# librosa/librosa

Measured on NVIDIA H100. Metric: mel-spectrogram frames/sec (n_fft=2048,hop=512,n_mels=128), higher is better.
Workload: dtype f32

## Files before the change

include/b2l.h:

```cpp
#ifndef B2L_H_
#define B2L_H_

#include <stddef.h>
#include <stdint.h>

#ifdef __cplusplus
extern "C" {
#endif

#define B2L_VERSION 100

enum b2l_status {
  B2L_OK = 0,
  B2L_ERR_INVALID = 1,
  B2L_ERR_CUDA = 2,
  B2L_ERR_UNSUPPORTED = 3,
  B2L_ERR_OOM = 4,
  B2L_ERR_NCCL = 5
};

enum b2l_pad_mode {
  B2L_PAD_CONSTANT = 0,
  B2L_PAD_EDGE = 1,
  B2L_PAD_REFLECT = 2,
// ... 30 lines not shown
int b2l_ctx_destroy(b2l_ctx* ctx);
int b2l_ctx_sync(b2l_ctx* ctx);
int b2l_ctx_device(const b2l_ctx* ctx, int* device);
int b2l_ctx_sm_count(const b2l_ctx* ctx, int* sms);
int b2l_ctx_launch_count(const b2l_ctx* ctx, uint64_t* launches);

int b2l_status_reset(b2l_ctx* ctx);
int b2l_status_read(b2l_ctx* ctx, int* status);
int b2l_scan_finite(b2l_ctx* ctx, const float* d_y, int64_t n_clips, int64_t n, int64_t y_stride,
                    int64_t begin);
int b2l_scan_finite_f64(b2l_ctx* ctx, const double* d_y, int64_t n_clips, int64_t n, int64_t y_stride,
                        int64_t begin);

int b2l_alloc(b2l_ctx* ctx, size_t bytes, void** d_ptr);
int b2l_free(b2l_ctx* ctx, void* d_ptr);
int b2l_memset(b2l_ctx* ctx, void* d_ptr, int value, size_t bytes);
int b2l_h2d(b2l_ctx* ctx, void* d_dst, const void* h_src, size_t bytes);
int b2l_d2h(b2l_ctx* ctx, void* h_dst, const void* d_src, size_t bytes);
int b2l_d2d(b2l_ctx* ctx, void* d_dst, const void* d_src, size_t bytes);
int b2l_copy2d(b2l_ctx* ctx, void* d_dst, size_t dst_pitch, const void* d_src, size_t src_pitch, size_t width_bytes,
               size_t rows);
int b2l_host_alloc(size_t bytes, void** h_ptr);
int b2l_host_free(void* h_ptr);
int b2l_mem_info(b2l_ctx* ctx, size_t* free_bytes, size_t* total_bytes);

int b2l_event_create(b2l_ctx* ctx, b2l_event** ev);
int b2l_event_record(b2l_ctx* ctx, b2l_event* ev);
int b2l_event_elapsed_ms(b2l_event* start, b2l_event* stop, float* ms);
int b2l_event_destroy(b2l_event* ev);

int b2l_plan_create(b2l_ctx* ctx, const b2l_plan_desc* desc, b2l_plan** plan);
int b2l_plan_destroy(b2l_plan* plan);
int b2l_plan_n_frames(const b2l_plan* plan, int64_t n, int64_t* n_frames);


int b2l_stft(b2l_ctx* ctx, const b2l_plan* plan, const float* d_y, int64_t n_clips, int64_t n,
             int64_t y_stride, void* d_D );

int b2l_spectrogram(b2l_ctx* ctx, const b2l_plan* plan, const float* d_y, int64_t n_clips, int64_t n,
                    int64_t y_stride, float* d_S);

int b2l_melspectrogram(b2l_ctx* ctx, const b2l_plan* plan, const float* d_y, int64_t n_clips, int64_t n,
                       int64_t y_stride, float* d_mel);

int b2l_mfcc(b2l_ctx* ctx, const b2l_plan* plan, const float* d_y, int64_t n_clips, int64_t n,
             int64_t y_stride, float* d_mfcc, float* d_logmel);

int b2l_istft(b2l_ctx* ctx, const b2l_plan* plan, const void* d_D, int64_t n_clips, int64_t n_frames_stored,
              int64_t n_frames_used, const float* d_inv_wss, int64_t out_len, float* d_y, int64_t y_stride);

int b2l_mel_project(b2l_ctx* ctx, const b2l_plan* plan, const float* d_S, int64_t n_clips,
                    int64_t n_frames, float* d_mel);
int b2l_power_to_db(b2l_ctx* ctx, const float* d_in, int64_t n_clips, int64_t per_clip, float amin,
                    float ref_value, float top_db, float* d_out);
typedef struct b2l_onset_desc {
  int32_t lag, max_size, pad_width, detrend, n_channels;
  int32_t bounds[33];
} b2l_onset_desc;
int b2l_onset_from_spec(b2l_ctx* ctx, const b2l_onset_desc* desc, const float* d_S, int64_t n_clips, int64_t n_rows,
                        int64_t n_frames, float* d_out);
int b2l_onset_median_from_spec(b2l_ctx* ctx, const b2l_onset_desc* desc, const float* d_S, int64_t n_clips,
                               int64_t n_rows, int64_t n_frames, float* d_out);
typedef struct b2l_pcen_desc {
  float gain, bias, power, eps, b;
  int32_t max_size;
} b2l_pcen_desc;
// ... 193 lines not shown
```

librosa_b200/_native.py:

```python
from __future__ import annotations

import ctypes as C
import os
import threading
import weakref
from typing import Optional, Tuple

import numpy as np

_HERE = os.path.dirname(os.path.abspath(__file__))
LIB_PATH = os.environ.get("B2L_LIB_PATH") or os.path.join(_HERE, "csrc", "libb2l.so")

B2L_OK = 0
B2L_ERR_INVALID = 1
B2L_ERR_CUDA = 2
B2L_ERR_UNSUPPORTED = 3
B2L_ERR_OOM = 4
B2L_ERR_NCCL = 5

PAD_MODES = {"constant": 0, "edge": 1, "reflect": 2, "symmetric": 3, "linear_ramp": 4, "empty": 5}


class NativeLibraryError(RuntimeError):
    """libb2l.so is missing / failed, or a CUDA / NCCL call failed."""
# ... 130 lines not shown
def _declare(lib):
    P = C.POINTER
    sig = {
        "b2l_version": (C.c_int, []),
        "b2l_last_error": (C.c_char_p, []),
        "b2l_device_count": (C.c_int, [P(C.c_int)]),
        "b2l_ctx_create": (C.c_int, [C.c_int, P(_vp)]),
        "b2l_ctx_destroy": (C.c_int, [_vp]),
        "b2l_ctx_sync": (C.c_int, [_vp]),
        "b2l_ctx_device": (C.c_int, [_vp, P(C.c_int)]),
        "b2l_ctx_sm_count": (C.c_int, [_vp, P(C.c_int)]),
        "b2l_ctx_launch_count": (C.c_int, [_vp, P(C.c_uint64)]),
        "b2l_status_reset": (C.c_int, [_vp]),
        "b2l_status_read": (C.c_int, [_vp, P(C.c_int)]),
        "b2l_scan_finite": (C.c_int, [_vp, _vp, _i64, _i64, _i64, _i64]),
        "b2l_scan_finite_f64": (C.c_int, [_vp, _vp, _i64, _i64, _i64, _i64]),
        "b2l_alloc": (C.c_int, [_vp, C.c_size_t, P(_vp)]),
        "b2l_free": (C.c_int, [_vp, _vp]),
        "b2l_memset": (C.c_int, [_vp, _vp, C.c_int, C.c_size_t]),
        "b2l_h2d": (C.c_int, [_vp, _vp, _vp, C.c_size_t]),
        "b2l_d2h": (C.c_int, [_vp, _vp, _vp, C.c_size_t]),
        "b2l_d2d": (C.c_int, [_vp, _vp, _vp, C.c_size_t]),
        "b2l_copy2d": (C.c_int, [_vp, _vp, C.c_size_t, _vp, C.c_size_t, C.c_size_t, C.c_size_t]),
        "b2l_host_alloc": (C.c_int, [C.c_size_t, P(_vp)]),
        "b2l_host_free": (C.c_int, [_vp]),
        "b2l_mem_info": (C.c_int, [_vp, P(C.c_size_t), P(C.c_size_t)]),
        "b2l_event_create": (C.c_int, [_vp, P(_vp)]),
        "b2l_event_record": (C.c_int, [_vp, _vp]),
        "b2l_event_elapsed_ms": (C.c_int, [_vp, _vp, P(C.c_float)]),
        "b2l_event_destroy": (C.c_int, [_vp]),
        "b2l_plan_create": (C.c_int, [_vp, P(PlanDesc), P(_vp)]),
        "b2l_plan_destroy": (C.c_int, [_vp]),
        "b2l_plan_n_frames": (C.c_int, [_vp, _i64, P(_i64)]),
        "b2l_stft": (C.c_int, [_vp, _vp, _vp, _i64, _i64, _i64, _vp]),
        "b2l_spectrogram": (C.c_int, [_vp, _vp, _vp, _i64, _i64, _i64, _vp]),
        "b2l_melspectrogram": (C.c_int, [_vp, _vp, _vp, _i64, _i64, _i64, _vp]),
        "b2l_mfcc": (C.c_int, [_vp, _vp, _vp, _i64, _i64, _i64, _vp, _vp]),
        "b2l_istft": (C.c_int, [_vp, _vp, _vp, _i64, _i64, _i64, _vp, _i64, _vp, _i64]),
        "b2l_mel_project": (C.c_int, [_vp, _vp, _vp, _i64, _i64, _vp]),
        "b2l_power_to_db": (C.c_int, [_vp, _vp, _i64, _i64, C.c_float, C.c_float, C.c_float, _vp]),
        "b2l_onset_from_spec": (C.c_int, [_vp, P(OnsetDesc), _vp, _i64, _i64, _i64, _vp]),
        "b2l_onset_median_from_spec": (C.c_int, [_vp, P(OnsetDesc), _vp, _i64, _i64, _i64, _vp]),
        "b2l_pcen": (C.c_int, [_vp, P(PcenDesc), _vp, _i64, _i64, _i64, _vp, _vp, _vp, _vp]),
        "b2l_resample_poly": (C.c_int, [_vp, _vp, _i64, _i64, _i64, _vp, C.c_int32, C.c_int32, C.c_int32, _i64, _i64, _i64,
                                        C.c_float, _vp]),
        "b2l_spectral_contrast": (C.c_int, [_vp, P(ContrastDesc), _vp, _i64, _i64, C.c_int32, _vp, _vp]),
        "b2l_sub": (C.c_int, [_vp, _vp, _vp, _i64, _vp]),
        "b2l_pip_pass": (C.c_int, [_vp, P(PipDesc), _vp, _i64, C.c_int32, _vp, _vp]),
        "b2l_normalize_rows": (C.c_int, [_vp, _vp, _i64, _i64, _i64, C.c_int32, C.c_float, _vp]),
        "b2l_hpss": (C.c_int, [_vp, P(HpssDesc), _vp, _vp, _i64, _i64, _i64, _vp, _vp]),
        "b2l_cabs": (C.c_int, [_vp, _vp, _i64, _vp]),
        "b2l_reassign": (C.c_int, [_vp, P(ReassignDesc), _vp, _vp, _vp, _i64, _i64, _i64, _vp, _vp, _vp, _vp, _vp]),
        "b2l_phase_vocoder": (C.c_int, [_vp, _vp, _i64, _i64, _i64, _i64, _vp, _vp, _vp, _vp, _vp]),
        "b2l_unary": (C.c_int, [_vp, C.c_int32, _vp, _i64, C.c_float, _vp]),
        "b2l_dct_project": (C.c_int, [_vp, _vp, _vp, _i64, _i64, _vp]),
        "b2l_transpose": (C.c_int, [_vp, _vp, _i64, _i64, _i64, C.c_int32, _vp]),
        "b2l_gl_update": (C.c_int, [_vp, _vp, _vp, _vp, C.c_float, C.c_float, _vp, _i64]),
        "b2l_spectral_stats": (C.c_int, [_vp, _vp, P(StatsDesc), _vp, _i64, _i64, _i64, _vp, _vp]),
        "b2l_spectral_stats_from_spec": (C.c_int, [_vp, P(StatsDesc), _vp, _i64, _i64, C.c_int32, _vp, _vp]),
        "b2l_frame_feature": (C.c_int, [_vp, C.c_int32, _vp, _i64, _i64, _i64, C.c_int32, C.c_int32, C.c_int32,
                                        C.c_int32, C.c_float, C.c_int32, C.c_int32, C.c_float, _vp]),
        "b2l_yin_cmnd": (C.c_int, [_vp, P(YinDesc), _vp, _i64, _i64, _i64, _vp]),
        "b2l_yin_pick": (C.c_int, [_vp, P(YinDesc), _vp, _i64, _vp]),
        "b2l_pyin_obs": (C.c_int, [_vp, P(PyinDesc), _vp, _i64, _vp, _vp, _vp, _vp]),
        "b2l_viterbi": (C.c_int, [_vp, P(PyinDesc), _vp, _vp, _vp, _vp, _i64, _i64, _vp, _vp, _vp]),
        "b2l_tempogram": (C.c_int, [_vp, P(TempogramDesc), _vp, _i64, _i64, _vp, _vp]),
# ... 447 lines not shown
```

librosa_b200/csrc/api.cu:

```cuda
#include <cuda_runtime.h>
#include <math.h>
#include <stdlib.h>
#include <string.h>

#include <algorithm>

#include "aux_kernels.cuh"
#include "czt_kernel.cuh"
#include "feat_kernels.cuh"
#include "internal.h"
#include "mr_kernel.cuh"
#include "pitch_kernels.cuh"

using namespace b2l;

#define B2L_CASE(L) case L: return fwd_kernel_##L(variant, mode);
static FwdKernel fwd_kernel_for(int log2m, int variant, int mode) {
  switch (log2m) { B2L_FFT_SIZES(B2L_CASE) }
  return nullptr;
}
#undef B2L_CASE
#define B2L_CASE(L) case L: return inv_kernel_##L(variant);
static InvKernel inv_kernel_for(int log2m, int variant) {
  switch (log2m) { B2L_FFT_SIZES(B2L_CASE) }
  return nullptr;
}
#undef B2L_CASE
#define B2L_CASE(L) case L: return czt_kernel_##L();
static CztKernel czt_kernel_for(int log2p) {
  switch (log2p) { B2L_CZT_SIZES(B2L_CASE) }
  return nullptr;
}
#undef B2L_CASE
#define B2L_CASE(L) case L: return czt_inv_kernel_##L();
static CztInvKernel czt_inv_kernel_for(int log2p) {
  switch (log2p) { B2L_CZT_SIZES(B2L_CASE) }
  return nullptr;
}
#undef B2L_CASE

static int cta_variants(const HostFftCfg& cfg, int out[3]) {
  int n = 0;
  if (cfg.log2m >= 9 && cfg.log2m <= 11) out[n++] = 116;
  int nws[2];
  const int k = cfg.nw_options(nws);
  for (int i = 0; i < k; ++i) out[n++] = nws[i];
  return n;
}
static int variant_threads(int variant) { return variant == 116 ? 512 : variant * 32; }

// ... 79 lines not shown
    off += (size_t)a.in_stride * nh;
    a.off_xbuf = (int)(off = align_up(off, 128));
    size_t xbytes = (size_t)f * cfg.xbuf_f2() * 8;
    if (mode == MODE_MEL || mode == MODE_STATS) {
      xbytes = (size_t)f * mel_group_stride(M, f) * 8 + (M < 128 ? (size_t)(M + 16) * 4 : 0);
    }
    a.xbuf_stride = (int)align_up(xbytes, 128);
    off += (size_t)a.xbuf_stride * nh;
    if (off > c->smem_optin) continue;
    variant = v;
    ft = f;
    halves = nh;
    smem = off;
    rt = t;
    a.in_floats = (int)span;
  }
  if (!variant)
    return fail(B2L_ERR_UNSUPPORTED, "hop_length=%d with n_fft=%d needs more shared memory than one SM has", p->hop,
                p->n_fft);

  a.y = d_y;
  a.clip_stride = y_stride;
  a.n = (int)n;
  a.n_clips = (int)n_clips;
  a.n_fft = N;
  a.hop = p->hop;
  a.pad = p->center ? N / 2 : 0;
  a.pad_mode = p->pad_mode;
  a.n_frames = (int)T;
  a.tiles_per_clip = (int)((T + ft - 1) / ft);
  a.total_tiles = (long long)a.tiles_per_clip * n_clips;
  a.tma_ok = (((uintptr_t)d_y & 15) == 0) && (y_stride % 4 == 0) && (a.in_floats % 4 == 0);
  a.window = p->d_win_fwd;
  a.tw = p->d_tw_fwd;
  a.twn = p->d_twn;
  a.out_c = out_c;
  a.out_r = out_r;
  a.power_mode = p->power_mode;
  a.power = p->power;
  a.n_mels = p->n_mels;
  if (mode == MODE_STATS) {
    if (!stats || !stats->d_freq) return fail(B2L_ERR_INVALID, "NULL frequency table");
    a.power_mode = 1;
    a.power = 1.0f;
    a.stats = stats->sp;
    a.mel_w = stats->d_freq;
    a.mel_w_count = M + 1;
  }
  if (rt) {
    a.mel_w_count = rt->w_count;
    a.mel_w = rt->d_w;
    a.mel_rows = rt->d_rows;
    a.n_mel_rows = rt->n_rows;
  }
  a.log_mode = log_mode ? 1 : 0;
  a.out_tiled = log_mode == 2 ? 1 : 0;
  a.amin = p->amin;
  a.db_sub = 10.0f * log10f(fmaxf(p->amin, fabsf(p->ref_value)));
  a.clip_max = c->d_clip_max;
  a.status = c->d_status;

  const FwdKernel fn = fwd_kernel_for(p->log2m, variant, mode);
  if (!fn) return fail(B2L_ERR_CUDA, "no forward kernel variant %d for n_fft=%d", variant, N);
  const int threads = variant_threads(variant);
  long long grid = 0;
  if ((rc = resident_grid(c, fn, threads, smem, (a.total_tiles + halves - 1) / halves, &grid))) return rc;
  if (!grid) return fail(B2L_ERR_CUDA, "forward kernel does not fit on an SM (smem %zu)", smem);
  return launch(c, fn, (unsigned)grid, threads, smem, a);
}

static size_t czt_smem(const b2l_plan* p, const HostFftCfg& cfg, int G, bool forward) {
  const size_t bins = forward ? (size_t)(1 + p->n_fft / 2) : 0;
  return (size_t)((cfg.tw_count() + 15) & ~15) * 8 + (size_t)G * cfg.xbuf_f2() * 8 +
         ((size_t)(1 << p->log2p) + (size_t)((p->n_fft + 1) & ~1) + bins) * 8;
}

static int run_czt(b2l_ctx* c, const b2l_plan* p, int mode, const float* d_y, int64_t n_clips, int64_t n,
                   int64_t y_stride, float2* out_c, float* out_r) {
  long long T = 0;
  int rc = frame_count(c, p, n_clips, n, y_stride, d_y, mode == 0 ? (void*)out_c : (void*)out_r, &T);
  if (rc || T == 0) return rc;
  DeviceGuard g(c->device);
  HostFftCfg cfg(p->log2p);
  const int nw = cfg.czt_nw();
  const int G = nw * 32 / cfg.tpf;
  CztArgs a;
  memset(&a, 0, sizeof(a));
  a.y = d_y;
  a.clip_stride = y_stride;
  a.n = (int)n;
  a.n_clips = (int)n_clips;
  a.L = p->n_fft;
  a.hop = p->hop;
  a.pad = p->center ? p->n_fft / 2 : 0;
  a.pad_mode = p->pad_mode;
// ... 1019 lines not shown
```

librosa_b200/csrc/common.cuh:

```cuda
#pragma once
#include <cuda_runtime.h>
#include <stdint.h>

namespace b2l {

enum PadMode : int {
  PAD_CONSTANT = 0,
  PAD_EDGE = 1,
  PAD_REFLECT = 2,
  PAD_SYMMETRIC = 3,
  PAD_LINEAR_RAMP = 4,
  PAD_EMPTY = 5,
};

enum FwdMode : int {
  MODE_STFT = 0,
  MODE_MEL = 1,
  MODE_SPEC = 2,
  MODE_STATS = 3,
};

constexpr int kMrMaxPass = 12;

struct MelBand { int lo, len, off, pad; };
// ... 6 lines not shown
  static constexpr int H = 32 / FP;
  static constexpr int RSM = H < 4 ? 4 : H;
  static constexpr int XB = M + M / 32;
  static constexpr int GS = XB + ((((RSM - 2 * XB) % 32) + 32) % 32) / 2;
  static constexpr int RS = 2 * GS;
  static_assert(RS >= M + 4 && RS % 32 == RSM % 32 && RS % 4 == 0, "row stride");
};
__host__ __device__ inline int mel_rows_per_warp(int ft) { return 32 / (((ft % 2) == 0 && ft >= 8) ? ft / 2 : ft); }
__host__ __device__ inline int mel_group_stride(int m, int ft) {
  const int h = mel_rows_per_warp(ft), rsm = h < 4 ? 4 : h, xb = m + m / 32;
  return xb + ((((rsm - 2 * xb) % 32) + 32) % 32) / 2;
}

enum StatRow : int { STAT_CENTROID = 0, STAT_BANDWIDTH = 1, STAT_ROLLOFF = 2, STAT_FLATNESS = 3, STAT_RMS = 4, STAT_TOTAL = 5 };
constexpr int N_STATS = 6;
struct StatsParams {
  float roll_percent;
  float flat_amin, flat_power;
  float bw_p;
  int bw_norm;
  int frame_length;
  int want;
};

struct FwdArgs {
  const float* y;
  long long clip_stride;
  int n, n_clips;
  int n_fft, hop, pad, pad_mode, n_frames;
  int tiles_per_clip;
  long long total_tiles;
  int tma_ok;
  const float* window;
  const float2* tw;
  const float2* twn;
  float2* out_c;
  float* out_r;
  int power_mode;
  float power;
  int n_mels, mel_w_count;
  const float* mel_w;
  const MelRow* mel_rows;
  int n_mel_rows;
  int log_mode;
  int out_tiled;
  float amin, db_sub;
  unsigned int* clip_max;
  int* status;
  StatsParams stats;
  int off_win, off_tw, off_in, off_xbuf, off_melw, off_melband, off_bar;
  int in_stride, xbuf_stride;
  int in_floats;
};

struct InvArgs {
  const float2* D;
  long long d_clip_stride;
  int n_clips, n_frames;
  int n_fft, hop, start;
  int out_len;
  long long y_clip_stride;
  float* y;
  const float* window;
  const float* inv_wss;
  const float2* tw;
  const float2* twn;
// ... 26 lines not shown
```

librosa_b200/csrc/fft_engine.cuh:

```cuda
#pragma once
#include <cuda_runtime.h>
#include <stdint.h>
#include <type_traits>
#include <utility>

namespace b2l {

template <int I, int N, class F>
__device__ __forceinline__ void static_for(F&& f) {
  if constexpr (I < N) {
    f(std::integral_constant<int, I>{});
    static_for<I + 1, N>(static_cast<F&&>(f));
  }
}

__host__ __device__ constexpr int ilog2c(int x) { return x <= 1 ? 0 : 1 + ilog2c(x >> 1); }
__host__ __device__ constexpr int bitrevc(int x, int bits) {
  int r = 0;
  for (int i = 0; i < bits; ++i) r |= ((x >> i) & 1) << (bits - 1 - i);
  return r;
}

constexpr double kPi = 3.14159265358979323846264338327950288;
constexpr double taylor_sin(double x) {
// ... 154 lines not shown
template <class Cfg, class LoadX, class Win>
__device__ __forceinline__ void load_pass0_windowed(float2 (&v)[Cfg::PPT], int t, LoadX&& load_x, Win&& win) {
  constexpr int R = Cfg::radix(0), LOGR = Cfg::log_radix(0), T = Cfg::M / R, NB = Cfg::PPT / R;
  static_assert(R >= 2, "fused first stage needs a radix of at least 2");
  static_for<0, NB>([&](auto B) {
    constexpr int b = decltype(B)::value;
    const int i = t + Cfg::TPF * b;
    static_for<0, R / 2>([&](auto J) {
      constexpr int j = decltype(J)::value;
      constexpr int sa = b * R + 2 * j, sb = sa + 1;
      constexpr int ra = bitrevc(2 * j, LOGR), rb = bitrevc(2 * j + 1, LOGR);
      const float2 xa = load_x(i + ra * T), xb = load_x(i + rb * T);
      const float2 wa = win(std::integral_constant<int, sa>{}), wb = win(std::integral_constant<int, sb>{});
      const float2 pw = mul2(xa, wa);
      v[sa] = fma2(xb, wb, pw);
      v[sb] = fma2(neg2(xb), wb, pw);
    });
  });
}

template <class Cfg>
__host__ __device__ constexpr int pass0_offset(int slot) {
  constexpr int R = Cfg::radix(0), LOGR = Cfg::log_radix(0), T = Cfg::M / R;
  return Cfg::TPF * (slot / R) + bitrevc(slot % R, LOGR) * T;
}
template <class Cfg>
__host__ __device__ constexpr int pass0_slot_of_pair(int c) {
  for (int s = 0; s < Cfg::PPT; ++s)
    if (pass0_offset<Cfg>(s) == Cfg::TPF * c) return s;
  return -1;
}

struct NoHook { __device__ __forceinline__ void operator()() const {} };
template <class Cfg, bool FUSED0 = false, bool SPLIT_TW = false, class Pre = NoHook>
__device__ __forceinline__ void fft_forward(float2 (&v)[Cfg::PPT], int t, int barrier_id, float2* __restrict__ xbuf,
                                            const float2* __restrict__ tw, Pre&& pre_store = Pre()) {
  constexpr int M = Cfg::M, TPF = Cfg::TPF, PPT = Cfg::PPT;
  static_for<0, Cfg::NPASS>([&](auto S) {
    constexpr int s = decltype(S)::value;
    constexpr int R = Cfg::radix(s);
    constexpr int LOGR = Cfg::log_radix(s);
    constexpr int p = Cfg::sublen(s);
    constexpr int T = M / R;
    constexpr int NB = PPT / R;
    constexpr bool SPLIT = SPLIT_TW && tw_split_pass(Cfg::LOG2M, s, R);
    const float2* tws = tw + Cfg::tw_offset(s, SPLIT_TW);
    constexpr bool AFFINE_LD = s > 0 && (TPF % 32 == 0) && (T % 32 == 0);
    const float2* ld_base = xbuf + xphys(t);
    static_for<0, NB>([&](auto B) {
      constexpr int b = decltype(B)::value;
      const int i = t + TPF * b;
      const float2* twk = tws + (i & (p - 1));
      float2 wlo[kTwSplitLo];
      if constexpr (SPLIT) {
        static_for<1, kTwSplitLo>([&](auto L) {
          constexpr int lo = decltype(L)::value;
          wlo[lo] = twk[(lo - 1) * p];
        });
      }
      static_for<0, R>([&](auto Rr) {
        constexpr int r = decltype(Rr)::value;
        constexpr int slot = b * R + bitrevc(r, LOGR);
        if constexpr (s > 0) {
          float2 x;
          if constexpr (AFFINE_LD) {
            constexpr int D = TPF * b + r * T;
            x = ld_base[D + D / 32];
          } else {
            x = xbuf[xphys(i + r * T)];
          }
          if constexpr (r > 0) {
            constexpr int lo = r % kTwSplitLo, hi = r / kTwSplitLo;
            if constexpr (!SPLIT) {
              x = cmul(x, twk[(r - 1) * p]);
            } else if constexpr (hi == 0) {
              x = cmul(x, wlo[lo]);
            } else if constexpr (lo == 0) {
              x = cmul(x, twk[(kTwSplitLo - 2 + hi) * p]);
            } else {
              x = cmul(x, cmul(twk[(kTwSplitLo - 2 + hi) * p], wlo[lo]));
            }
          }
          v[slot] = x;
        }
      });
    });
    static_for<0, NB>([&](auto B) { dft_reg<R, decltype(B)::value * R, (FUSED0 && s == 0) ? 1 : 0>(v); });
    if constexpr (s + 1 < Cfg::NPASS) {
      if constexpr (s > 0) group_sync<TPF>(barrier_id);
      else pre_store();
      constexpr bool AFFINE_ST = (TPF % 32 == 0) && (R == 32 ? true : false) && (p == 1 || p % 32 == 0) && ((TPF * R) % 32 == 0) &&
                                 (p == 1 ? (R % 32 == 0) : true) && (TPF % p == 0 || p == 1);
      if constexpr (AFFINE_ST) {
        const int k0 = t & (p - 1);
        const uint32_t st_base = smem_u32(xbuf + xphys((t - k0) * R + k0));
        static_for<0, NB>([&](auto B) {
          constexpr int b = decltype(B)::value;
          static_for<0, R>([&](auto Q) {
            constexpr int q = decltype(Q)::value;
            constexpr int D = TPF * b * R + q * p;
            sts_c64(st_base + 8u * (D + D / 32), v[b * R + q]);
          });
        });
      } else {
        static_for<0, NB>([&](auto B) {
          constexpr int b = decltype(B)::value;
          const int i = t + TPF * b;
          const int k = i & (p - 1);
          const int j = (i - k) * R + k;
          const uint32_t xbuf_s = smem_u32(xbuf);
          static_for<0, R>([&](auto Q) {
            constexpr int q = decltype(Q)::value;
            sts_c64(xbuf_s + 8u * xphys(j + q * p), v[b * R + q]);
// ... 50 lines not shown
```

librosa_b200/csrc/fwd_inst.cu:

```cuda
#include "fwd_kernel.cuh"
#include "internal.h"

#ifndef B2L_LOG2M
#error "compile with -DB2L_LOG2M=<2..12>"
#endif

namespace b2l {
namespace {

template <int L, int TPF, int NW, int DUAL>
FwdKernel by_mode(int mode) {
  switch (mode) {
    case MODE_STFT: return fwd_kernel<L, TPF, NW, MODE_STFT, DUAL>;
    case MODE_MEL: return fwd_kernel<L, TPF, NW, MODE_MEL, DUAL>;
    case MODE_SPEC: return fwd_kernel<L, TPF, NW, MODE_SPEC, DUAL>;
    case MODE_STATS: return fwd_kernel<L, TPF, NW, MODE_STATS, DUAL>;
  }
  return nullptr;
}

template <int L>
FwdKernel variant_kernel(int variant, int mode) {
  constexpr int M = 1 << L;
  constexpr int TPF = M >= 32 ? M / 32 : 1;
  if constexpr (L >= 10) {
    if (variant == 16) return by_mode<L, TPF, 16, 1>(mode);
    if (variant == 8) return by_mode<L, TPF, 8, 1>(mode);
    if (variant == 116) return by_mode<L, TPF, 16, 2>(mode);
  } else {
    constexpr int NW = TPF > 16 ? 16 : TPF;
    if (variant == NW) return by_mode<L, TPF, NW, 1>(mode);
    if constexpr (L == 9) {
      if (variant == 116) return by_mode<L, TPF, 16, 2>(mode);
    }
  }
  return nullptr;
}

}

#define B2L_CAT2(a, b) a##b
#define B2L_CAT(a, b) B2L_CAT2(a, b)

FwdKernel B2L_CAT(fwd_kernel_, B2L_LOG2M)(int variant, int mode) { return variant_kernel<B2L_LOG2M>(variant, mode); }

}
```

librosa_b200/csrc/fwd_kernel.cuh:

```cuda
#pragma once
#include "common.cuh"
#include "fft_engine.cuh"
#include "stats.cuh"


namespace b2l {

__device__ __forceinline__ void mbar_init(uint64_t* bar, int count) {
  asm volatile("mbarrier.init.shared::cta.b64 [%0], %1;" ::"r"(smem_u32(bar)), "r"(count) : "memory");
}
__device__ __forceinline__ void fence_mbar_init() {
  asm volatile("fence.mbarrier_init.release.cluster;" ::: "memory");
}
__device__ __forceinline__ void fence_proxy_async() {
  asm volatile("fence.proxy.async.shared::cta;" ::: "memory");
}
__device__ __forceinline__ void mbar_expect_tx(uint64_t* bar, uint32_t bytes) {
  asm volatile("mbarrier.arrive.expect_tx.shared::cta.b64 _, [%0], %1;" ::"r"(smem_u32(bar)), "r"(bytes)
               : "memory");
}
__device__ __forceinline__ void mbar_wait(uint64_t* bar, uint32_t phase) {
  asm volatile(
      "{\n\t"
      ".reg .pred p;\n\t"
// ... 43 lines not shown
    default:
      return 0.0f;
  }
}

static __device__ __noinline__ float power_from_sq(float p2, int power_mode, float power) {
  float mag = sqrtf(p2);
  return power_mode == 1 ? mag : powf(mag, power);
}
__device__ __forceinline__ float sqmag(float2 x) { return fmaf(x.x, x.x, x.y * x.y); }
__device__ __forceinline__ float db10(float x) { return 3.0102999566398120f * __log2f(x); }
__device__ __forceinline__ float sqrt_approx(float x) {
  float r;
  asm("sqrt.approx.f32 %0, %1;" : "=f"(r) : "f"(x));
  return r;
}

template <int M, int TPF, int C>
__device__ __forceinline__ int partner_slot(int t) {
  if constexpr (TPF % 32 == 0) {
    constexpr int WPG = TPF / 32;
    const int tl = t & 31, tw = t >> 5;
    const int row = tw + WPG * C;
    const int rows = M / 32;
    const int a = 33 * (rows - 1 - row) + 32 - tl;
    const int b = 33 * ((rows - row) & (rows - 1));
    return tl == 0 ? b : a;
  } else {
    const int k = t + TPF * C;
    return xphys((M - k) & (M - 1));
  }
}

template <int LOG2M, int TPF, int NW, int MODE, int NSPLIT>
__global__ void __launch_bounds__(NW * 32, 1) fwd_kernel(const FwdArgs a) {
  using Cfg = FftCfg<LOG2M, TPF>;
  constexpr int M = Cfg::M, N = 2 * M, PPT = Cfg::PPT;
  constexpr int NT = NW * 32;
  constexpr int NH = NSPLIT;
  constexpr bool DUAL = NSPLIT > 1;
  constexpr int HT = NT / NH;
  constexpr int HW = NW / NH;
  constexpr int FT = HT / TPF;
  static_assert(NW % NSPLIT == 0, "the warps are split evenly");
  static_assert(TPF <= 32 || NH + NT / TPF <= 15, "named barriers: 1..NH for the halves, then one per frame group");
  static_assert(FT >= 1 && FT <= 32, "tile must hold 1..32 frames");
  using ML = MelLayout<M, FT>;
  constexpr int H = ML::H;
  constexpr int NPAIR = PPT / 2;

  extern __shared__ __align__(128) unsigned char smem[];
  const int tid = threadIdx.x;
  const int half = DUAL ? tid / HT : 0;
  const int htid = tid - half * HT;
  float* s_win = reinterpret_cast<float*>(smem + a.off_win);
  float2* s_tw = reinterpret_cast<float2*>(smem + a.off_tw);
  float* s_melw = reinterpret_cast<float*>(smem + a.off_melw);
  MelRow* s_row = reinterpret_cast<MelRow*>(smem + a.off_melband);
  float* s_in = reinterpret_cast<float*>(smem + a.off_in + half * a.in_stride);
  float2* s_xall = reinterpret_cast<float2*>(smem + a.off_xbuf + half * a.xbuf_stride);
  float* s_p = reinterpret_cast<float*>(s_xall);
  uint64_t* s_bar = reinterpret_cast<uint64_t*>(smem + a.off_bar) + half;

  const int grp = htid / TPF;
  const int t = htid % TPF;
  const int gbar = 1 + NH + half * FT + grp;
  constexpr int GS = (MODE == MODE_MEL || MODE == MODE_STATS) ? ML::GS : Cfg::XBUF_F2;
  float2* xbuf = s_xall + grp * GS;
  float2* xb_t = xbuf + xphys(t);
  const float2* xb_neg = xbuf - xphys(t) + ((t & 31) == 0 ? 1 : 0);

  auto half_sync = [&]() {
    if constexpr (DUAL) asm volatile("bar.sync %0, %1;" ::"r"(half + 1), "n"(HT) : "memory");
    else __syncthreads();
  };

  for (int i = tid; i < N; i += NT) s_win[i] = a.window[i];
  for (int i = tid; i < Cfg::TW_COUNT_SPLIT; i += NT) s_tw[i] = a.tw[i];
  if constexpr (MODE == MODE_MEL) {
    for (int i = tid; i < a.mel_w_count; i += NT) s_melw[i] = a.mel_w[i];
    for (int i = tid; i < a.n_mel_rows; i += NT) s_row[i] = a.mel_rows[i];
  }
  if constexpr (MODE == MODE_STATS) {
    for (int i = tid; i < a.mel_w_count; i += NT) s_melw[i] = a.mel_w[i];
  }
  if (htid == 0) {
    mbar_init(s_bar, 1);
    fence_mbar_init();
  }
  __syncthreads();

  const int span = a.in_floats;
  const bool hop_even = (a.hop & 1) == 0;
  const float2 wt = __ldg(a.twn + t);
  auto unmix_tw = [&](auto C) -> float2 {
    constexpr int c = decltype(C)::value;
    if constexpr (c == 0) return wt;
    else return cmul(wt, make_float2(TwC<c, 2 * PPT>::re, TwC<c, 2 * PPT>::im));
  };

  enum { TILE_GATHER = 0, TILE_TMA = 1, TILE_TMA_ZERO = 2 };
  struct TileInfo { int clip, tix, kind, lead, valid; };
  auto describe = [&](int clip, int tix) -> TileInfo {
    TileInfo ti;
    ti.clip = clip;
    ti.tix = tix;
    const long long s0 = (long long)tix * FT * a.hop - a.pad;
    ti.lead = s0 < 0 ? (int)(-s0) : 0;
    const long long end = s0 + span;
    ti.valid = (int)((end > a.n ? (long long)a.n : end) - (s0 + ti.lead));
// ... 10 lines not shown
      mbar_expect_tx(s_bar, (uint32_t)ti.valid * 4u);
      tma_load_1d(s_in + ti.lead, a.y + (long long)ti.clip * a.clip_stride + s0 + ti.lead, (uint32_t)ti.valid * 4u, s_bar);
    }
    if (ti.clip < a.n_clips && ti.kind == TILE_TMA_ZERO) {
      for (int i = htid; i < ti.lead; i += HT) s_in[i] = 0.0f;
      for (int i = ti.lead + ti.valid + htid; i < span; i += HT) s_in[i] = 0.0f;
    }
  };

  const int tile_step = (int)gridDim.x * NH;
  const int step_c = tile_step / a.tiles_per_clip, step_t = tile_step - step_c * a.tiles_per_clip;
  TileInfo cur;
  {
    const int first = (int)blockIdx.x * NH + half;
    cur = describe(first / a.tiles_per_clip, first % a.tiles_per_clip);
  }
  uint32_t phase = 0;
  prefetch(cur);

  constexpr bool ROWS = (MODE == MODE_MEL || MODE == MODE_STATS);
  float2 v[PPT];
  auto stage_and_fetch = [&](const TileInfo& ti) {
    if (ti.kind == TILE_GATHER) {
      const float* yc = a.y + (long long)ti.clip * a.clip_stride;
      const long long s0 = (long long)ti.tix * FT * a.hop - a.pad;
      for (int i = htid; i < span; i += HT) s_in[i] = load_padded(yc, a.n, s0 + i, a.pad_mode, a.pad);
      half_sync();
    } else {
      mbar_wait(s_bar, phase);
      phase ^= 1;
      if (ti.kind == TILE_TMA_ZERO) half_sync();
    }
    const float* fr = s_in + grp * a.hop;
    auto win = [&](auto S) {
      constexpr int off = pass0_offset<Cfg>(decltype(S)::value);
      return *reinterpret_cast<const float2*>(s_win + 2 * (t + off));
    };
    if (hop_even) {
      load_pass0_windowed<Cfg>(v, t, [&](int e) { return *reinterpret_cast<const float2*>(fr + 2 * e); }, win);
    } else {
      load_pass0_windowed<Cfg>(v, t, [&](int e) { return make_float2(fr[2 * e], fr[2 * e + 1]); }, win);
    }
  };
  auto advance = [&](const TileInfo& ti) -> TileInfo {
    int nc = ti.clip + step_c, nt = ti.tix + step_t;
    if (nt >= a.tiles_per_clip) { nt -= a.tiles_per_clip; ++nc; }
    return describe(nc, nt);
  };

  for (; cur.clip < a.n_clips;) {
    const int clip = cur.clip, t0 = cur.tix * FT;
    stage_and_fetch(cur);
    const TileInfo nxt = advance(cur);
    half_sync();
    prefetch(nxt);
    auto rows_consumed = [&]() {
      if constexpr (ROWS) half_sync();
    };

    fft_forward<Cfg, true, true>(v, t, gbar, xbuf, s_tw, rows_consumed);
    if constexpr (Cfg::NPASS == 1) rows_consumed();
    constexpr bool SHFL_UNMIX = TPF == 32 && (MODE == MODE_MEL || MODE == MODE_STATS);
    static_assert(!SHFL_UNMIX || (PPT == 32 && spectrum_offset<Cfg>(1) == 32), "v[q] = Z[t + 32q]");
    constexpr bool AFFINE_UNMIX = (TPF % 32 == 0) && (TPF > 32 || MODE == MODE_MEL || MODE == MODE_STATS);
    if constexpr (!SHFL_UNMIX) {
      if constexpr (Cfg::NPASS > 1) group_sync<TPF>(gbar);
      static_for<0, PPT>([&](auto S) {
        constexpr int slot = decltype(S)::value;
        constexpr int D = spectrum_offset<Cfg>(slot);
        if constexpr (D >= M / 2) {
          if constexpr (AFFINE_UNMIX && D % 32 == 0) sts_c64(smem_u32(xb_t) + 8u * (D + D / 32), v[slot]);
          else sts_c64(smem_u32(xbuf) + 8u * xphys(t + D), v[slot]);
        }
      });
      group_sync<TPF>(gbar);
    }
    auto pair_operands = [&](auto C, float2& A, float2& B) {
      constexpr int c = decltype(C)::value;
      constexpr int sa = slot_of_pair<Cfg>(c);
      static_assert(sa >= 0, "pair operand must be register resident");
      A = v[sa];
      if constexpr (SHFL_UNMIX) {
        const float2 send = t == 0 ? v[(32 - c) & 31] : v[31 - c];
        B.x = __shfl_sync(0xffffffffu, send.x, (32 - t) & 31);
        B.y = __shfl_sync(0xffffffffu, send.y, (32 - t) & 31);
      } else if constexpr (AFFINE_UNMIX) {
        constexpr int K = 33 * (M / 32 - 1 - (TPF / 32) * c) + 32;
        if constexpr (c == 0) B = t == 0 ? A : xb_neg[K];
        else B = xb_neg[K];
      } else {
        B = xbuf[partner_slot<M, TPF, c>(t)];
        if constexpr (c == 0) {
          if (t == 0) B = A;
// ... 167 lines not shown
```

librosa_b200/csrc/internal.h:

```cpp
#pragma once
#include <cuda_runtime.h>
#include <stdint.h>

#include <algorithm>
#include <map>
#include <set>
#include <tuple>
#include <vector>

#include "../../include/b2l.h"
#include "common.cuh"
#include "fft_engine.cuh"

namespace b2l {

#define B2L_FFT_SIZES(X) X(2) X(3) X(4) X(5) X(6) X(7) X(8) X(9) X(10) X(11) X(12)
#define B2L_CZT_SIZES(X) X(5) X(6) X(7) X(8) X(9) X(10) X(11) X(12)
constexpr int kMinLog2M = 2, kMaxLog2M = 12;

struct CztArgs;
struct CztInvArgs;
typedef void (*FwdKernel)(FwdArgs);
typedef void (*InvKernel)(InvArgs);
typedef void (*CztKernel)(CztArgs);
typedef void (*CztInvKernel)(CztInvArgs);

#define B2L_DECL_FFT(L) FwdKernel fwd_kernel_##L(int variant, int mode); InvKernel inv_kernel_##L(int variant);
#define B2L_DECL_CZT(L) CztKernel czt_kernel_##L(); CztInvKernel czt_inv_kernel_##L();
B2L_FFT_SIZES(B2L_DECL_FFT)
B2L_CZT_SIZES(B2L_DECL_CZT)
#undef B2L_DECL_FFT
#undef B2L_DECL_CZT

struct HostFftCfg {
  int log2m, M, tpf, ppt, logp, npass;
  explicit HostFftCfg(int l2m) {
    log2m = l2m;
    M = 1 << l2m;
    tpf = M >= 32 ? M / 32 : 1;
    ppt = M / tpf;
    logp = 0;
    while ((1 << logp) < ppt) ++logp;
    npass = ppt == 1 ? 1 : (log2m + logp - 1) / logp;
  }
  int log_radix(int s) const { int left = log2m - s * logp; return left >= logp ? logp : left; }
  int radix(int s) const { return 1 << log_radix(s); }
  int sublen(int s) const { return 1 << (s * logp); }
  bool split_pass(int s, bool split) const { return split && tw_split_pass(log2m, s, radix(s)); }
  int tw_rows(int s, bool split) const { return split_pass(s, split) ? kTwSplitRows : radix(s) - 1; }
  int tw_offset(int s, bool split = false) const {
    int off = 0;
    for (int q = 1; q < s; ++q) off += tw_rows(q, split) * sublen(q);
    return off;
  }
  int tw_count(bool split = false) const { return tw_offset(npass, split); }
  int xbuf_f2() const { return M + M / 32; }
  int czt_nw() const { return log2m >= 10 ? 16 : (tpf > 16 ? 16 : tpf); }
  int nw_options(int out[2]) const {
    if (log2m >= 10) { out[0] = 16; out[1] = 8; return 2; }
    out[0] = tpf >= 1 ? (tpf > 16 ? 16 : tpf) : 1;
// ... 9 lines not shown
    if (_e != cudaSuccess) {                                                                  \
      cudaGetLastError();                                                                     \
      return fail(_e == cudaErrorMemoryAllocation ? B2L_ERR_OOM : B2L_ERR_CUDA, "%s: %s (%s:%d)", #expr, \
                  cudaGetErrorString(_e), __FILE__, __LINE__);                                \
    }                                                                                         \
  } while (0)

}

struct b2l_ctx {
  int device = 0;
  int sm_count = 0;
  size_t smem_optin = 0;
  cudaStream_t stream = nullptr;
  uint64_t launches = 0;
  struct ncclComm* comm = nullptr;
  int rank = 0, world = 1;
  unsigned int* d_clip_max = nullptr;
  int* d_status = nullptr;
  float* d_scratch = nullptr;
  size_t scratch_bytes = 0;
  size_t clip_max_cap = 0;
  std::set<const void*> smem_limit_set;
  std::map<std::tuple<const void*, int, size_t>, int> occupancy;
  std::vector<void*> stage_bufs;
  std::vector<cudaEvent_t> stage_evs;
};

struct b2l_plan {
  b2l_ctx* ctx = nullptr;
  int n_fft = 0, hop = 0, center = 0, pad_mode = 0, log2m = 0;
  mutable std::vector<void*> allocs;
  float* d_win_fwd = nullptr;
  float* d_win_inv = nullptr;
  float2* d_tw = nullptr;
  float2* d_tw_fwd = nullptr;
  float2* d_twn = nullptr;
  int tw_count = 0;
  int n_mels = 0, mel_w_count = 0;
  float* d_mel_w = nullptr;
  b2l::MelBand* d_band = nullptr;
  float* d_mel_wT = nullptr;
  std::vector<b2l::MelBand> h_band;
  std::vector<float> h_mel_w;
  struct RowTable { b2l::MelRow* d_rows = nullptr; float* d_w = nullptr; int n_rows = 0, w_count = 0; };
  mutable std::map<int, RowTable> row_tables;
  int power_mode = 2;
  float power = 2.0f;
  int czt = 0, log2p = 0;
  float2* d_czt_wb = nullptr;
  float2* d_czt_bk = nullptr;
  float2* d_czt_hf = nullptr;
  float2* d_czt_bfull = nullptr;
  float2* d_czt_wbi = nullptr;
  int mr = 0, mr_n_pass = 0, mr_tw_count = 0;
  int mr_radix[b2l::kMrMaxPass] = {0}, mr_tw_off[b2l::kMrMaxPass] = {0};
  float* d_mr_win = nullptr;
  float* d_mr_win_inv = nullptr;
  float2* d_mr_tw = nullptr;
  float2* d_mr_twn = nullptr;
  int n_mfcc = 0;
  float* d_dct = nullptr;
  float amin = 1e-10f, ref_value = 1.0f, top_db = 80.0f;
};

namespace b2l {
// ... 87 lines not shown
```

librosa_b200/csrc/plan.cu:

```cuda
#include <cuda_runtime.h>
#include <math.h>

#include <algorithm>
#include <complex>
#include <vector>

#include "internal.h"

using namespace b2l;

template <class T>
static int upload(const b2l_plan* p, const std::vector<T>& h, T** d) {
  *d = nullptr;
  const size_t bytes = h.size() * sizeof(T);
  CUDA_TRY(cudaMalloc((void**)d, bytes ? bytes : 16));
  p->allocs.push_back(*d);
  if (bytes) CUDA_TRY(cudaMemcpy(*d, h.data(), bytes, cudaMemcpyHostToDevice));
  return B2L_OK;
}

std::vector<float2> b2l::engine_twiddles(const HostFftCfg& cfg, bool split) {
  const double two_pi = 6.283185307179586476925286766559;
  std::vector<float2> tw((size_t)cfg.tw_count(split));
  for (int s = 1; s < cfg.npass; ++s) {
// ... 21 lines not shown
  for (size_t len = 2; len <= n; len <<= 1) {
    for (size_t i = 0; i < n; i += len)
      for (size_t k = 0; k < len / 2; ++k) {
        const double ang = -2.0 * kPi * (double)k / (double)len;
        const std::complex<double> w(cos(ang), sin(ang));
        const std::complex<double> u = x[i + k], v = x[i + k + len / 2] * w;
        x[i + k] = u + v;
        x[i + k + len / 2] = u - v;
      }
  }
}

static std::vector<float2> unmix_twiddles(int N) {
  std::vector<float2> twn((size_t)N / 4 + 1);
  for (int k = 0; k <= N / 4; ++k) {
    const double ang = -2.0 * kPi * (double)k / (double)N;
    twn[k] = make_float2((float)cos(ang), (float)sin(ang));
  }
  return twn;
}

static bool mr_factor(int n_fft, std::vector<int>& radices) {
  radices.clear();
  if (n_fft < 12 || (n_fft & 1) || n_fft > 4096) return false;
  int m = n_fft / 2;
  while (m % 5 == 0) { radices.push_back(5); m /= 5; }
  while (m % 3 == 0) { radices.push_back(3); m /= 3; }
  while (m % 8 == 0) { radices.push_back(8); m /= 8; }
  if (m % 4 == 0) { radices.push_back(4); m /= 4; }
  if (m % 2 == 0) { radices.push_back(2); m /= 2; }
  return m == 1 && (int)radices.size() <= kMrMaxPass && !radices.empty();
}

static int build_pow2(b2l_plan* p, const double* window) {
  const int N = p->n_fft;
  HostFftCfg cfg(p->log2m);
  std::vector<float> wf(N), wi(N);
  for (int i = 0; i < N; ++i) {
    wf[i] = (float)(window[i] * 0.5);
    wi[i] = (float)(window[i] / (double)N);
  }
  p->tw_count = cfg.tw_count();
  int rc;
  if ((rc = upload(p, wf, &p->d_win_fwd)) || (rc = upload(p, wi, &p->d_win_inv)) ||
      (rc = upload(p, engine_twiddles(cfg), &p->d_tw)) || (rc = upload(p, engine_twiddles(cfg, true), &p->d_tw_fwd)) ||
      (rc = upload(p, unmix_twiddles(N), &p->d_twn)))
    return rc;
  return B2L_OK;
}

static int build_czt(b2l_plan* p, const double* window) {
  const int L = p->n_fft, P = 1 << p->log2p;
  std::vector<std::complex<double>> b(L);
  for (int n = 0; n < L; ++n) {
    const long long q = ((long long)n * n) % (2LL * L);
    const double ang = -kPi * (double)q / (double)L;
    b[n] = std::complex<double>(cos(ang), sin(ang));
  }
  std::vector<float2> wb(L), bk(L / 2 + 1);
  for (int n = 0; n < L; ++n) {
    const std::complex<double> z = window[n] * b[n];
    wb[n] = make_float2((float)z.real(), (float)z.imag());
  }
  for (int k = 0; k <= L / 2; ++k) bk[k] = make_float2((float)b[k].real(), (float)b[k].imag());
  std::vector<std::complex<double>> h(P, std::complex<double>(0.0, 0.0));
  h[0] = std::conj(b[0]);
  for (int m = 1; m < L; ++m) h[m] = h[P - m] = std::conj(b[m]);
  host_fft(h);
  std::vector<float2> hf((size_t)P);
// ... 236 lines not shown
```

Baseline: 311.8 million.

## Compute cosine-sum window analytically and derive split twiddles in registers

At plan time the window is tested for the form a0 - a1*cos(2πk/N), which covers Hann and Hamming. When it matches, forward kernels stop loading the window table into shared memory and instead evaluate each window sample from the per-thread twiddle with compile-time constants and FMAs. For n_fft=2048 with row-streaming modes (including mel), the split-twiddle factors of the first FFT pass are built in registers from powers of one complex value rather than read from the shared table. Both trade shared-memory loads for extra arithmetic, and repeated complex multiplies in float32 add small rounding error; the new template flag also doubles the number of kernel instantiations.

```diff
diff --git a/include/b2l.h b/include/b2l.h
--- a/include/b2l.h
+++ b/include/b2l.h
@@ -86,6 +86,7 @@
 int b2l_plan_create(b2l_ctx* ctx, const b2l_plan_desc* desc, b2l_plan** plan);
 int b2l_plan_destroy(b2l_plan* plan);
 int b2l_plan_n_frames(const b2l_plan* plan, int64_t n, int64_t* n_frames);
+int b2l_window_cosine_sum(const double* h_window, int32_t n, int32_t* is_cosine, double* a0, double* a1);
 
 
 int b2l_stft(b2l_ctx* ctx, const b2l_plan* plan, const float* d_y, int64_t n_clips, int64_t n,
diff --git a/librosa_b200/_native.py b/librosa_b200/_native.py
--- a/librosa_b200/_native.py
+++ b/librosa_b200/_native.py
@@ -186,6 +186,7 @@
         "b2l_plan_create": (C.c_int, [_vp, P(PlanDesc), P(_vp)]),
         "b2l_plan_destroy": (C.c_int, [_vp]),
         "b2l_plan_n_frames": (C.c_int, [_vp, _i64, P(_i64)]),
+        "b2l_window_cosine_sum": (C.c_int, [P(C.c_double), C.c_int32, P(C.c_int32), P(C.c_double), P(C.c_double)]),
         "b2l_stft": (C.c_int, [_vp, _vp, _vp, _i64, _i64, _i64, _vp]),
         "b2l_spectrogram": (C.c_int, [_vp, _vp, _vp, _i64, _i64, _i64, _vp]),
         "b2l_melspectrogram": (C.c_int, [_vp, _vp, _vp, _i64, _i64, _i64, _vp]),
diff --git a/librosa_b200/csrc/api.cu b/librosa_b200/csrc/api.cu
--- a/librosa_b200/csrc/api.cu
+++ b/librosa_b200/csrc/api.cu
@@ -14,8 +14,8 @@
 
 using namespace b2l;
 
-#define B2L_CASE(L) case L: return fwd_kernel_##L(variant, mode);
-static FwdKernel fwd_kernel_for(int log2m, int variant, int mode) {
+#define B2L_CASE(L) case L: return fwd_kernel_##L(variant, mode, win_cos);
+static FwdKernel fwd_kernel_for(int log2m, int variant, int mode, bool win_cos) {
   switch (log2m) { B2L_FFT_SIZES(B2L_CASE) }
   return nullptr;
 }
@@ -161,6 +161,8 @@
   a.total_tiles = (long long)a.tiles_per_clip * n_clips;
   a.tma_ok = (((uintptr_t)d_y & 15) == 0) && (y_stride % 4 == 0) && (a.in_floats % 4 == 0);
   a.window = p->d_win_fwd;
+  a.win_a0 = p->win_a0;
+  a.win_a1 = p->win_a1;
   a.tw = p->d_tw_fwd;
   a.twn = p->d_twn;
   a.out_c = out_c;
@@ -189,7 +191,7 @@
   a.clip_max = c->d_clip_max;
   a.status = c->d_status;
 
-  const FwdKernel fn = fwd_kernel_for(p->log2m, variant, mode);
+  const FwdKernel fn = fwd_kernel_for(p->log2m, variant, mode, p->win_cos);
   if (!fn) return fail(B2L_ERR_CUDA, "no forward kernel variant %d for n_fft=%d", variant, N);
   const int threads = variant_threads(variant);
   long long grid = 0;
diff --git a/librosa_b200/csrc/common.cuh b/librosa_b200/csrc/common.cuh
--- a/librosa_b200/csrc/common.cuh
+++ b/librosa_b200/csrc/common.cuh
@@ -62,6 +62,7 @@
   long long total_tiles;
   int tma_ok;
   const float* window;
+  float win_a0, win_a1;
   const float2* tw;
   const float2* twn;
   float2* out_c;
diff --git a/librosa_b200/csrc/fft_engine.cuh b/librosa_b200/csrc/fft_engine.cuh
--- a/librosa_b200/csrc/fft_engine.cuh
+++ b/librosa_b200/csrc/fft_engine.cuh
@@ -210,9 +210,10 @@
 }
 
 struct NoHook { __device__ __forceinline__ void operator()() const {} };
-template <class Cfg, bool FUSED0 = false, bool SPLIT_TW = false, class Pre = NoHook>
+template <class Cfg, bool FUSED0 = false, bool SPLIT_TW = false, class Pre = NoHook, bool REG_TW = false>
 __device__ __forceinline__ void fft_forward(float2 (&v)[Cfg::PPT], int t, int barrier_id, float2* __restrict__ xbuf,
-                                            const float2* __restrict__ tw, Pre&& pre_store = Pre()) {
+                                            const float2* __restrict__ tw, Pre&& pre_store = Pre(),
+                                            float2 wk = make_float2(1.0f, 0.0f)) {
   constexpr int M = Cfg::M, TPF = Cfg::TPF, PPT = Cfg::PPT;
   static_for<0, Cfg::NPASS>([&](auto S) {
     constexpr int s = decltype(S)::value;
@@ -230,7 +231,19 @@
       const int i = t + TPF * b;
       const float2* twk = tws + (i & (p - 1));
       float2 wlo[kTwSplitLo];
-      if constexpr (SPLIT) {
+      float2 whi[32 / kTwSplitLo];
+      if constexpr (SPLIT && REG_TW) {
+        wlo[1] = wk;
+        wlo[2] = cmul(wk, wk);
+        wlo[3] = cmul(wlo[2], wk);
+        wlo[4] = cmul(wlo[2], wlo[2]);
+        wlo[5] = cmul(wlo[4], wk);
+        wlo[6] = cmul(wlo[3], wlo[3]);
+        wlo[7] = cmul(wlo[4], wlo[3]);
+        whi[1] = cmul(wlo[4], wlo[4]);
+        whi[2] = cmul(whi[1], whi[1]);
+        whi[3] = cmul(whi[2], whi[1]);
+      } else if constexpr (SPLIT) {
         static_for<1, kTwSplitLo>([&](auto L) {
           constexpr int lo = decltype(L)::value;
           wlo[lo] = twk[(lo - 1) * p];
@@ -254,9 +267,9 @@
             } else if constexpr (hi == 0) {
               x = cmul(x, wlo[lo]);
             } else if constexpr (lo == 0) {
-              x = cmul(x, twk[(kTwSplitLo - 2 + hi) * p]);
+              x = cmul(x, REG_TW ? whi[hi] : twk[(kTwSplitLo - 2 + hi) * p]);
             } else {
-              x = cmul(x, cmul(twk[(kTwSplitLo - 2 + hi) * p], wlo[lo]));
+              x = cmul(x, cmul(REG_TW ? whi[hi] : twk[(kTwSplitLo - 2 + hi) * p], wlo[lo]));
             }
           }
           v[slot] = x;
diff --git a/librosa_b200/csrc/fwd_inst.cu b/librosa_b200/csrc/fwd_inst.cu
--- a/librosa_b200/csrc/fwd_inst.cu
+++ b/librosa_b200/csrc/fwd_inst.cu
@@ -8,30 +8,37 @@
 namespace b2l {
 namespace {
 
-template <int L, int TPF, int NW, int DUAL>
+template <int L, int NW, int DUAL>
+constexpr bool stft_keeps_table() { return (L == 9 && DUAL == 2) || (L == 11 && NW == 16 && DUAL == 1); }
+
+template <int L, int TPF, int NW, int DUAL, bool WIN_COS>
 FwdKernel by_mode(int mode) {
   switch (mode) {
-    case MODE_STFT: return fwd_kernel<L, TPF, NW, MODE_STFT, DUAL>;
-    case MODE_MEL: return fwd_kernel<L, TPF, NW, MODE_MEL, DUAL>;
-    case MODE_SPEC: return fwd_kernel<L, TPF, NW, MODE_SPEC, DUAL>;
-    case MODE_STATS: return fwd_kernel<L, TPF, NW, MODE_STATS, DUAL>;
+    case MODE_STFT: return fwd_kernel<L, TPF, NW, MODE_STFT, DUAL, WIN_COS && !stft_keeps_table<L, NW, DUAL>()>;
+    case MODE_MEL: return fwd_kernel<L, TPF, NW, MODE_MEL, DUAL, WIN_COS>;
+    case MODE_SPEC: return fwd_kernel<L, TPF, NW, MODE_SPEC, DUAL, WIN_COS>;
+    case MODE_STATS: return fwd_kernel<L, TPF, NW, MODE_STATS, DUAL, WIN_COS>;
   }
   return nullptr;
 }
+template <int L, int TPF, int NW, int DUAL>
+FwdKernel by_mode(int mode, bool win_cos) {
+  return win_cos ? by_mode<L, TPF, NW, DUAL, true>(mode) : by_mode<L, TPF, NW, DUAL, false>(mode);
+}
 
 template <int L>
-FwdKernel variant_kernel(int variant, int mode) {
+FwdKernel variant_kernel(int variant, int mode, bool win_cos) {
   constexpr int M = 1 << L;
   constexpr int TPF = M >= 32 ? M / 32 : 1;
   if constexpr (L >= 10) {
-    if (variant == 16) return by_mode<L, TPF, 16, 1>(mode);
-    if (variant == 8) return by_mode<L, TPF, 8, 1>(mode);
-    if (variant == 116) return by_mode<L, TPF, 16, 2>(mode);
+    if (variant == 16) return by_mode<L, TPF, 16, 1>(mode, win_cos);
+    if (variant == 8) return by_mode<L, TPF, 8, 1>(mode, win_cos);
+    if (variant == 116) return by_mode<L, TPF, 16, 2>(mode, win_cos);
   } else {
     constexpr int NW = TPF > 16 ? 16 : TPF;
-    if (variant == NW) return by_mode<L, TPF, NW, 1>(mode);
+    if (variant == NW) return by_mode<L, TPF, NW, 1>(mode, win_cos);
     if constexpr (L == 9) {
-      if (variant == 116) return by_mode<L, TPF, 16, 2>(mode);
+      if (variant == 116) return by_mode<L, TPF, 16, 2>(mode, win_cos);
     }
   }
   return nullptr;
@@ -42,6 +49,8 @@
 #define B2L_CAT2(a, b) a##b
 #define B2L_CAT(a, b) B2L_CAT2(a, b)
 
-FwdKernel B2L_CAT(fwd_kernel_, B2L_LOG2M)(int variant, int mode) { return variant_kernel<B2L_LOG2M>(variant, mode); }
+FwdKernel B2L_CAT(fwd_kernel_, B2L_LOG2M)(int variant, int mode, bool win_cos) {
+  return variant_kernel<B2L_LOG2M>(variant, mode, win_cos);
+}
 
 }
diff --git a/librosa_b200/csrc/fwd_kernel.cuh b/librosa_b200/csrc/fwd_kernel.cuh
--- a/librosa_b200/csrc/fwd_kernel.cuh
+++ b/librosa_b200/csrc/fwd_kernel.cuh
@@ -99,7 +99,7 @@
   }
 }
 
-template <int LOG2M, int TPF, int NW, int MODE, int NSPLIT>
+template <int LOG2M, int TPF, int NW, int MODE, int NSPLIT, bool WIN_COS>
 __global__ void __launch_bounds__(NW * 32, 1) fwd_kernel(const FwdArgs a) {
   using Cfg = FftCfg<LOG2M, TPF>;
   constexpr int M = Cfg::M, N = 2 * M, PPT = Cfg::PPT;
@@ -142,7 +142,8 @@
     else __syncthreads();
   };
 
-  for (int i = tid; i < N; i += NT) s_win[i] = a.window[i];
+  if constexpr (!WIN_COS)
+    for (int i = tid; i < N; i += NT) s_win[i] = a.window[i];
   for (int i = tid; i < Cfg::TW_COUNT_SPLIT; i += NT) s_tw[i] = a.tw[i];
   if constexpr (MODE == MODE_MEL) {
     for (int i = tid; i < a.mel_w_count; i += NT) s_melw[i] = a.mel_w[i];
@@ -219,14 +220,32 @@
       if (ti.kind == TILE_TMA_ZERO) half_sync();
     }
     const float* fr = s_in + grp * a.hop;
-    auto win = [&](auto S) {
-      constexpr int off = pass0_offset<Cfg>(decltype(S)::value);
-      return *reinterpret_cast<const float2*>(s_win + 2 * (t + off));
+    auto fetch = [&](auto win) {
+      if (hop_even) {
+        load_pass0_windowed<Cfg>(v, t, [&](int e) { return *reinterpret_cast<const float2*>(fr + 2 * e); }, win);
+      } else {
+        load_pass0_windowed<Cfg>(v, t, [&](int e) { return make_float2(fr[2 * e], fr[2 * e + 1]); }, win);
+      }
     };
-    if (hop_even) {
-      load_pass0_windowed<Cfg>(v, t, [&](int e) { return *reinterpret_cast<const float2*>(fr + 2 * e); }, win);
+    if constexpr (WIN_COS) {
+      const float2 z = cmul(wt, wt);
+      const float C = -a.win_a1 * z.x, S = -a.win_a1 * z.y, A0 = a.win_a0;
+      auto wsample = [&](auto Mc) {
+        using Psi = TwC<decltype(Mc)::value, N>;
+        constexpr float c = Psi::re, s = -Psi::im;
+        if constexpr (s == 0.0f) return fmaf(C, c, A0);
+        else if constexpr (c == 0.0f) return fmaf(S, s, A0);
+        else return fmaf(S, s, fmaf(C, c, A0));
+      };
+      fetch([&](auto SL) {
+        constexpr int m = 2 * pass0_offset<Cfg>(decltype(SL)::value);
+        return make_float2(wsample(std::integral_constant<int, m>{}), wsample(std::integral_constant<int, m + 1>{}));
+      });
     } else {
-      load_pass0_windowed<Cfg>(v, t, [&](int e) { return make_float2(fr[2 * e], fr[2 * e + 1]); }, win);
+      fetch([&](auto SL) {
+        constexpr int off = pass0_offset<Cfg>(decltype(SL)::value);
+        return *reinterpret_cast<const float2*>(s_win + 2 * (t + off));
+      });
     }
   };
   auto advance = [&](const TileInfo& ti) -> TileInfo {
@@ -245,7 +264,8 @@
       if constexpr (ROWS) half_sync();
     };
 
-    fft_forward<Cfg, true, true>(v, t, gbar, xbuf, s_tw, rows_consumed);
+    if constexpr (LOG2M == 10 && ROWS) fft_forward<Cfg, true, true, decltype(rows_consumed)&, true>(v, t, gbar, xbuf, s_tw, rows_consumed, cmul(wt, wt));
+    else fft_forward<Cfg, true, true>(v, t, gbar, xbuf, s_tw, rows_consumed);
     if constexpr (Cfg::NPASS == 1) rows_consumed();
     constexpr bool SHFL_UNMIX = TPF == 32 && (MODE == MODE_MEL || MODE == MODE_STATS);
     static_assert(!SHFL_UNMIX || (PPT == 32 && spectrum_offset<Cfg>(1) == 32), "v[q] = Z[t + 32q]");
diff --git a/librosa_b200/csrc/internal.h b/librosa_b200/csrc/internal.h
--- a/librosa_b200/csrc/internal.h
+++ b/librosa_b200/csrc/internal.h
@@ -25,7 +25,7 @@
 typedef void (*CztKernel)(CztArgs);
 typedef void (*CztInvKernel)(CztInvArgs);
 
-#define B2L_DECL_FFT(L) FwdKernel fwd_kernel_##L(int variant, int mode); InvKernel inv_kernel_##L(int variant);
+#define B2L_DECL_FFT(L) FwdKernel fwd_kernel_##L(int variant, int mode, bool win_cos); InvKernel inv_kernel_##L(int variant);
 #define B2L_DECL_CZT(L) CztKernel czt_kernel_##L(); CztInvKernel czt_inv_kernel_##L();
 B2L_FFT_SIZES(B2L_DECL_FFT)
 B2L_CZT_SIZES(B2L_DECL_CZT)
@@ -101,6 +101,8 @@
   int n_fft = 0, hop = 0, center = 0, pad_mode = 0, log2m = 0;
   mutable std::vector<void*> allocs;
   float* d_win_fwd = nullptr;
+  int win_cos = 0;
+  float win_a0 = 0.0f, win_a1 = 0.0f;
   float* d_win_inv = nullptr;
   float2* d_tw = nullptr;
   float2* d_tw_fwd = nullptr;
diff --git a/librosa_b200/csrc/plan.cu b/librosa_b200/csrc/plan.cu
--- a/librosa_b200/csrc/plan.cu
+++ b/librosa_b200/csrc/plan.cu
@@ -77,9 +77,37 @@
   return m == 1 && (int)radices.size() <= kMrMaxPass && !radices.empty();
 }
 
+static bool cosine_window(const double* w, int n, double* a0, double* a1) {
+  if (n < 2 || (n & 1)) return false;
+  const double c0 = 0.5 * (w[0] + w[n / 2]), c1 = 0.5 * (w[n / 2] - w[0]);
+  double peak = 0.0;
+  for (int k = 0; k < n; ++k) peak = std::max(peak, fabs(w[k]));
+  const double tol = 1e-12 * peak;
+  for (int k = 0; k < n; ++k) {
+    const double model = c0 - c1 * cos(2.0 * kPi * (double)k / (double)n);
+    if (!(fabs(w[k] - model) <= tol)) return false;
+  }
+  *a0 = c0;
+  *a1 = c1;
+  return true;
+}
+
+extern "C" int b2l_window_cosine_sum(const double* h_window, int32_t n, int32_t* is_cosine, double* a0, double* a1) {
+  if (!h_window || !is_cosine || !a0 || !a1) return fail(B2L_ERR_INVALID, "NULL argument");
+  *a0 = *a1 = 0.0;
+  *is_cosine = cosine_window(h_window, n, a0, a1) ? 1 : 0;
+  return B2L_OK;
+}
+
 static int build_pow2(b2l_plan* p, const double* window) {
   const int N = p->n_fft;
   HostFftCfg cfg(p->log2m);
+  double a0, a1;
+  if (cosine_window(window, N, &a0, &a1)) {
+    p->win_cos = 1;
+    p->win_a0 = (float)(a0 * 0.5);
+    p->win_a1 = (float)(a1 * 0.5);
+  }
   std::vector<float> wf(N), wi(N);
   for (int i = 0; i < N; ++i) {
     wf[i] = (float)(window[i] * 0.5);
```

Result: faster. 316.6 million (median of 6 runs) (+1.5%).
